# HKPolyU-UAV/bluerov2

Hardware: AMD Instinct MI355X
Metric: NMPC RTI solves/s (N=20, 12 states / 4 inputs), batch 4096 per GPU (higher is better)
Workload: dtype f64; 1 GPU; BASELINE.json configs[1]: batch=4096 independent BlueROV2 NMPC instances per GPU, N=20, Ts=0.05 s, circle reference window advancing one row per step, per-instance x0 noise (seed 1), nominal parameters, default options (qp_early_exit=1: exact equality-constrained shortcut when no bound is active); batch_per_gpu=4096, N=20, parallelism=single GPU

## Files before the change

bluerov2_amd/csrc/lin_device.hpp:

```cpp
#pragma once
#include "bluerov2_model.hpp"
#include "nmpc_device.hpp"

namespace brov {

__device__ __forceinline__ void kkt_upd(double& kkt, double v) {
    const double a = fabs(v);
    kkt = (a != a) ? a : ((kkt != kkt) ? kkt : fmax(kkt, a));
}

struct KktAcc {
    double mx = 0.0;
    bool nan = false;
    __device__ __forceinline__ void upd(double v) { mx = fmax(mx, fabs(v)); nan = nan || (v != v); }
};

__device__ __forceinline__ void rk4_state(const double* __restrict__ xi, const Wrench& w, const ModelPar& m, double h,
                                          StagePoint (&sp)[4], double (&xn)[NX]) {
    double x[NX], k[NX], xs[NX];
#pragma unroll
    for (int j = 0; j < NX; j++) x[j] = xi[j];
    model_f(x, w, m, k, sp[0]);
#pragma unroll
    for (int j = 0; j < NX; j++) { xn[j] = x[j] + (h / 6.0) * k[j]; xs[j] = x[j] + 0.5 * h * k[j]; }
// ... 107 lines not shown
    jvp_rec2(R, m.imx, m.imy, m.imz, m.imn, s0, s1, k0, k1);
#pragma unroll
    for (int st = 1; st < 4; st++) {
        R = load_stage_rec(rec + st * kRecStage);
        __builtin_amdgcn_sched_barrier(0);
        const double wprev = (st == 1) ? h / 6.0 : h / 3.0, cs = (st == 3) ? h : 0.5 * h;
#pragma unroll
        for (int j = 0; j < NX; j++) {
            const double e0 = (j == c0) ? 1.0 : 0.0, e1 = (j == c1) ? 1.0 : 0.0;
            acc0[j] = (st == 1 ? e0 : acc0[j]) + wprev * k0[j]; s0[j] = e0 + cs * k0[j];
            acc1[j] = (st == 1 ? e1 : acc1[j]) + wprev * k1[j]; s1[j] = e1 + cs * k1[j];
        }
        __builtin_amdgcn_sched_barrier(0);
        jvp_rec2(R, m.imx, m.imy, m.imz, m.imn, s0, s1, k0, k1);
    }
#pragma unroll
    for (int j = 0; j < NX; j++) { acc0[j] += (h / 6.0) * k0[j]; acc1[j] += (h / 6.0) * k1[j]; }
}

struct KktOperands { double pm1c, ll, lu, ucur, lbu, ubu, grad, qn; };
struct KktGlobal { double pm1c, ll, lu, ucur; };
__device__ __forceinline__ KktGlobal load_kkt_global(const DevParams& P, int b, int ig, int c, const double* __restrict__ ui) {
    const int N = P.N;
    const int jc = c - NX, ju = jc & 3, cx = c < NX ? c : NX - 1;
    const double* __restrict__ pim1 = P.pi + ((size_t)b * N + (ig > 0 ? ig - 1 : 0)) * NX;
    const double* __restrict__ lam = P.lam + ((size_t)b * N + ig) * 8;
    KktGlobal G;
    G.pm1c = pim1[cx];
    G.ll = lam[ju];
    G.lu = lam[4 + ju];
    G.ucur = ui[ju];
    return G;
}
__device__ __forceinline__ KktOperands finish_kkt_operands(const KktGlobal& G, const double* __restrict__ cst, int il, int nl, int c,
                                                           const lds_f64* q_s, const lds_f64* r_s) {
    const int jc = c - NX, ju = jc & 3, cx = c < NX ? c : NX - 1;
    KktOperands K;
    K.pm1c = G.pm1c; K.ll = G.ll; K.lu = G.lu; K.ucur = G.ucur;
    K.lbu = cst[32 + ju];
    K.ubu = cst[36 + ju];
    const lds_f64* gp = jc < 0 ? q_s + il * NX + c : r_s + il * NU + jc;
    K.grad = *gp;
    K.qn = q_s[nl * NX + cx];
    return K;
}
__device__ __forceinline__ KktOperands load_kkt_operands(const DevParams& P, const double* __restrict__ cst, int b, int ig, int il,
                                                         int nl, int c, const double* __restrict__ ui, const lds_f64* q_s,
                                                         const lds_f64* r_s) {
    return finish_kkt_operands(load_kkt_global(P, b, ig, c, ui), cst, il, nl, c, q_s, r_s);
}

__device__ __forceinline__ void sens_column_rec(const lds_f64* rec, const ModelPar& m, double h, int c, double (&acc)[NX]) {
    double ks[NX], ss[NX], kb[4];
    const int jc = c - NX;
    constexpr double ir = 1.0 / kRotor;
    kb[0] = jc == 0 ? (-4.0 * 0.707) * ir * m.imx : 0.0;
    kb[1] = jc == 1 ? (4.0 * 0.707) * ir * m.imy : 0.0;
    kb[2] = jc == 2 ? -2.0 * ir * m.imz : 0.0;
    kb[3] = jc == 1 ? (0.167 + 0.167 - 0.175 - 0.175) * ir * m.imn : (jc == 3 ? (0.167 + 0.167 + 0.175 + 0.175) * ir * m.imn : 0.0);
    StageRec R = load_stage_rec(rec);
    __builtin_amdgcn_sched_barrier(0);
#pragma unroll
    for (int j = 0; j < NX; j++) ss[j] = (j == c) ? 1.0 : 0.0;
    jvp_rec(R, m.imx, m.imy, m.imz, m.imn, kb, ss, ks);
    R = load_stage_rec(rec + kRecStage);
    __builtin_amdgcn_sched_barrier(0);
#pragma unroll
    for (int j = 0; j < NX; j++) { acc[j] = ((j == c) ? 1.0 : 0.0) + (h / 6.0) * ks[j]; ss[j] = ((j == c) ? 1.0 : 0.0) + 0.5 * h * ks[j]; }
    __builtin_amdgcn_sched_barrier(0);
    jvp_rec(R, m.imx, m.imy, m.imz, m.imn, kb, ss, ks);
    R = load_stage_rec(rec + 2 * kRecStage);
    __builtin_amdgcn_sched_barrier(0);
#pragma unroll
    for (int j = 0; j < NX; j++) { acc[j] += (h / 3.0) * ks[j]; ss[j] = ((j == c) ? 1.0 : 0.0) + 0.5 * h * ks[j]; }
    __builtin_amdgcn_sched_barrier(0);
    jvp_rec(R, m.imx, m.imy, m.imz, m.imn, kb, ss, ks);
    R = load_stage_rec(rec + 3 * kRecStage);
    __builtin_amdgcn_sched_barrier(0);
#pragma unroll
    for (int j = 0; j < NX; j++) { acc[j] += (h / 3.0) * ks[j]; ss[j] = ((j == c) ? 1.0 : 0.0) + h * ks[j]; }
    __builtin_amdgcn_sched_barrier(0);
    jvp_rec(R, m.imx, m.imy, m.imz, m.imn, kb, ss, ks);
// ... 116 lines not shown
```

bluerov2_amd/csrc/qp/fused.hpp:

```cpp
#pragma once

namespace brov {

constexpr int kFusedMaxN = 23;
template <int W, bool GRID, bool DF>
__device__ __forceinline__ bool rti_fused_step(const DevParams& P, int b, int lane, bool listed, size_t yoff) {
    extern __shared__ __attribute__((aligned(16))) double smem[];
    const int N = P.N;
    double* ba_s = smem;
    double* bv_s = ba_s + (size_t)N * kBaStage;
    double* kt_s = bv_s + (size_t)N * NX;
    double* kff_s = kt_s + (size_t)N * kKtStage;
    double* vh_s = kff_s + (size_t)N * 4;
    double* dx_s = vh_s + (size_t)N * 4;
    double* q_s = dx_s + (size_t)(N + 1) * NX;
    double* r_s = q_s + (size_t)(N + 1) * NX;
    double* const_s = r_s + (size_t)N * 4;
    if (lane == 0) { const_s[0] = 0.0; const_s[1] = 1.0; }
    LaneCst lc;
    if constexpr (W == 1) lc = load_lane_cst(P.cst, lane);
    double part = 0.0;
    bool nanp = false;
    lin_phase<W == 1, GRID>(P, b, 0, N, lane, ba_s, bv_s, kt_s, q_s, r_s, part, nanp, true, yoff);
    __syncthreads();
    if (P.dump_lin) copy_out_linearisation(P, b, 0, N, lane, ba_s, bv_s);
    std::conditional_t<GRID, InstGrid, Inst> I;
    setup_inst(P, I, b, lane, W == 1 ? &lc : nullptr, yoff);
    const bool listed_u = __builtin_amdgcn_readfirstlane((int)listed) != 0;
    I.ckpt = (N >= 8 && P.partial_refactor && listed_u) ? (N + 3) >> 2 : 0;
    I.lds_ba = (const lds_f64*)ba_s;
    I.lds_bv = (const lds_f64*)bv_s;
    I.lds_kt = (lds_f64*)kt_s;
    I.lds_q = (const lds_f64*)q_s;
    I.lds_r = (const lds_f64*)r_s;
    I.kff = kff_s;
    I.vhat = vh_s;
    I.dxb = dx_s;
    I.lds_kff = (lds_f64*)kff_s;
    I.lds_vhat = (lds_f64*)vh_s;
    I.lds_dxb = (lds_f64*)dx_s;
    I.lds_zero = (lds_f64*)const_s;
    I.lds_tr = (lds_f64*)const_s + 2;
    {
        const int rg = I.rg, cl = I.cl;
        const int zero = (int)(const_s - ba_s), one = zero + 1, kt0 = (int)(kt_s - ba_s);
        for (int r = 0; r < 3; r++) I.ba_off[r] = cl >= 3 ? (rg + 4 * r) * kBaStride + cl - 3 : ((r == 0 && rg == cl) ? one : zero);
        I.ba_str = cl >= 3 ? kBaStage : 0;
        for (int r = 0; r < 4; r++) {
            const int c = rg + 4 * r;
            I.bat_off[r] = cl >= NX ? zero : (c >= 3 ? cl * kBaStride + c - 3 : (c == cl ? one : zero));
        }
        I.bat_str = cl >= NX ? 0 : kBaStage;
        I.bat_str0 = (cl < NX && rg == 3) ? kBaStage : 0;
        for (int r = 0; r < 3; r++) I.kt_off[r] = cl < 4 ? kt0 + (rg + 4 * r) * 4 + cl : zero;
        I.kt_str = cl < 4 ? kKtStage : 0;
    }
    qp_body<W, std::conditional_t<GRID, InstGrid, Inst>, DF>(P, I, b, part, nanp);
    return I.ran_loop;
}
__device__ __forceinline__ void plant_step_wave(const DevParams& P, int b, int lane, int tk) {
    double x[NX], u[NU], k[NX], xs[NX], acc[NX];
    double* x0 = P.x0_rw + (size_t)b * NX;
#pragma unroll
    for (int j = 0; j < NX; j++) x[j] = x0[j];
#pragma unroll
    for (int j = 0; j < NU; j++) u[j] = P.res[b].u0[j];
    const ModelPar m = make_par(P.plant_pp + (size_t)b * NP);
    Wrench w = make_wrench(u);
    if (P.plant_rp) { w.k3 = P.plant_rp[(size_t)b * P.plant_rp_stride]; w.k4 = P.plant_rp[(size_t)b * P.plant_rp_stride + 1]; }
    const double h = P.plant_dt / P.plant_substeps;
    StagePoint sp;
    for (int s = 0; s < P.plant_substeps; s++) {
        model_f(x, w, m, k, sp);
#pragma unroll
        for (int j = 0; j < NX; j++) { acc[j] = x[j] + (h / 6.0) * k[j]; xs[j] = x[j] + 0.5 * h * k[j]; }
        model_f(xs, w, m, k, sp);
#pragma unroll
        for (int j = 0; j < NX; j++) { acc[j] += (h / 3.0) * k[j]; xs[j] = x[j] + 0.5 * h * k[j]; }
        model_f(xs, w, m, k, sp);
#pragma unroll
        for (int j = 0; j < NX; j++) { acc[j] += (h / 3.0) * k[j]; xs[j] = x[j] + h * k[j]; }
        model_f(xs, w, m, k, sp);
#pragma unroll
        for (int j = 0; j < NX; j++) x[j] = acc[j] + (h / 6.0) * k[j];
    }
    if (lane == 0) {
#pragma unroll
        for (int j = 0; j < NX; j++) x0[j] = x[j];
        if (P.plant_xlog) {
#pragma unroll
            for (int j = 0; j < NX; j++) P.plant_xlog[((size_t)tk * P.B + b) * NX + j] = x[j];
        }
        if (P.plant_ulog) {
#pragma unroll
            for (int j = 0; j < NU; j++) P.plant_ulog[((size_t)tk * P.B + b) * NU + j] = u[j];
        }
    }
}

template <int W, bool GRID = false, bool DF = false, bool MULTI = false>
__device__ __forceinline__ void rti_fused_body(const DevParams& P) {
    const int b = __builtin_amdgcn_readfirstlane(sched_map(P, blockIdx.x));
    const int lane = threadIdx.x;
    bool listed = sched_listed(P, b);
    if (blockIdx.x == 0) sched_zero_next(P, lane);
    DBG_STAMP(0);
    if constexpr (!MULTI) {
        (void)rti_fused_step<W, GRID, DF>(P, b, lane, listed, 0);
    } else {
#pragma clang loop unroll(disable)
        for (int tk = 0; tk < P.ticks; tk++) {
            int bq = b, lq = lane;
            asm volatile("s_mov_b32 %0, %0" : "+s"(bq));
            asm volatile("v_mov_b32 %0, %0" : "+v"(lq));
            listed = rti_fused_step<W, GRID, DF>(P, bq, lq, listed, (size_t)tk * (size_t)P.tick_yref);
            if (P.tick_status && lq == 0) P.tick_status[(size_t)tk * P.B + bq] = P.res[bq].status;
            __syncthreads();
            wave_fence();
            if (P.plant_pp) {
                plant_step_wave(P, bq, lq, tk);
                __syncthreads();
                wave_fence();
            }
        }
    }
}

}
```

bluerov2_amd/csrc/qp/lin_phase.hpp:

```cpp
#pragma once

namespace brov {

template <int MAXC>
__device__ __forceinline__ void stage_issue(const double* __restrict__ g, int nd, int lane, dbl2 (&v)[MAXC]) {
#pragma unroll
    for (int k = 0; k < MAXC; k++) {
        const int o = (lane + 64 * k) * 2;
        v[k] = *(const dbl2*)(g + (o < nd ? o : 0));
    }
}
template <int MAXC>
__device__ __forceinline__ void stage_store(double* l, int nd, int lane, const dbl2 (&v)[MAXC]) {
#pragma unroll
    for (int k = 0; k < MAXC; k++) {
        const int o = (lane + 64 * k) * 2;
        if (o < nd) *(lds_d2*)(l + o) = v[k];
    }
}

template <bool TWO = true, bool GRID = false>
__device__ __forceinline__ void lin_phase(const DevParams& P, int b, int i0, int n, int lane, double* ba_s, double* bv_s,
                                          double* rec_s, double* q_s, double* r_s, double& part, bool& nanp, bool stamp, size_t yoff = 0) {
#ifdef BROV_DBG_LIN
    unsigned long long lin_t[8] = {0, 0, 0, 0, 0, 0, 0, 0};
#endif
    const int N = P.N;
    const double* __restrict__ cst = P.cst;
    const int L = n <= 4 ? 16 : 64 / n;
    const int g = lane / L, j0 = lane - g * L;
    const bool active = g < n;
    const int i = active ? g : n - 1;
    const int ig = i0 + i;
    const double* __restrict__ ui = P.u + ((size_t)b * N + ig) * NU;
    const double hstep = GRID ? P.tsv[ig] : P.Ts;
    double rp0 = 0.0, rp1 = 0.0;
    if constexpr (TWO) {
        if (P.par_rp) { const double* rp = P.par_rp + ((size_t)b * (N + 1) + ig) * 2; rp0 = rp[0]; rp1 = rp[1]; }
    }
    const int po = i0 > 0 ? 1 : 0;
    double* sx = ba_s;
    double* spar = sx + (size_t)(n + 1) * NX;
    double* syr = spar + (size_t)n * NP;
    double* spi = syr + (size_t)(n + 1) * NY;
    double* su = spi + (size_t)(n + 1) * NX;
    {
        dbl2 vx[3], vp[3], vy[3], vpi[3], vu[1];
        stage_issue(P.x + ((size_t)b * (N + 1) + i0) * NX, (n + 1) * NX, lane, vx);
        stage_issue(P.par + ((size_t)b * (N + 1) + i0) * NP, n * NP, lane, vp);
        stage_issue(P.yref + yoff + (size_t)b * P.yref_stride + (size_t)i0 * NY, (n + 1) * NY, lane, vy);
        stage_issue(P.pi + ((size_t)b * N + i0 - po) * NX, (n + po) * NX, lane, vpi);
        stage_issue(P.u + ((size_t)b * N + i0) * NU, n * NU, lane, vu);
        stage_store(sx, (n + 1) * NX, lane, vx);
        stage_store(spar, n * NP, lane, vp);
        stage_store(syr, (n + 1) * NY, lane, vy);
        stage_store(spi, (n + po) * NX, lane, vpi);
        stage_store(su, n * NU, lane, vu);
    }
    const double* xi = sx + i * NX;
    const double* pp = spar + i * NP;
    const double* yr = syr + i * NY;
    const double* pil = spi + (i + po) * NX;
    const double* pim1 = spi + (ig > 0 ? i + po - 1 : 0) * NX;
    double uu[NU], x0r[NX], yrr[NY], pir[NX], pm1[3];
#pragma unroll
    for (int j = 0; j < NU; j++) uu[j] = su[i * NU + j];
#pragma unroll
    for (int j = 0; j < NX; j++) { x0r[j] = xi[j]; pir[j] = pil[j]; }
#pragma unroll
    for (int j = 0; j < NY; j++) yrr[j] = yr[j];
#pragma unroll
    for (int j = 0; j < 3; j++) pm1[j] = pim1[j];
    const unsigned long long tA = (stamp && P.dbg) ? __builtin_readcyclecounter() : 0;
    LIN_T(0);
    const bool last = ig == N - 1;
    double yrn[NX];
#pragma unroll
    for (int j = 0; j < NX; j++) yrn[j] = yr[NY + j];
    const ModelPar m = make_par(pp);
    Wrench w = make_wrench(uu);
    if constexpr (!TWO) {
        if (P.par_rp) { const double* rp = P.par_rp + ((size_t)b * (N + 1) + ig) * 2; rp0 = rp[0]; rp1 = rp[1]; }
    }
    w.k3 = rp0; w.k4 = rp1;
    KktAcc ka;
#pragma unroll
    for (int k = 0; k < NX; k++) {
        const double qk = (GRID ? P.wst[(size_t)ig * 16 + k] : P.Ts * cst[k]) * (x0r[k] - yrr[k]);
        q_s[i * NX + k] = qk;
        if (k < 3) ka.upd(ig >= 1 ? qk + pir[k] - pm1[k] : 0.0);
    }
#pragma unroll
    for (int k = 0; k < NU; k++) r_s[i * NU + k] = (GRID ? P.wst[(size_t)ig * 16 + NX + k] : P.Ts * cst[NX + k]) * (uu[k] - yrr[NX + k]);
    if (last) {
#pragma unroll
        for (int k = 0; k < NX; k++) {
            const double qn = cst[16 + k] * (xi[NX + k] - yrn[k]);
            q_s[n * NX + k] = qn;
            if (k < 3) ka.upd(qn - pir[k]);
        }
    }
    const unsigned long long tB = (stamp && P.dbg) ? __builtin_readcyclecounter() : 0;
    LIN_T(1);
    StagePoint sp[4];
    double xn[NX];
    rk4_state(x0r, w, m, hstep, sp, xn);
    const unsigned long long tC = (stamp && P.dbg) ? __builtin_readcyclecounter() : 0;
    LIN_T(2);
    double* tb = ba_s + i * kBaStage;
    lds_f64* rec = (lds_f64*)rec_s + i * kRecInterval;
#pragma unroll
    for (int st = 0; st < 4; st++) store_stage_rec(rec + st * kRecStage, sp[st], m);
#pragma unroll
    for (int k = 0; k < NX; k++) {
        const double bk = xn[k] - xi[NX + k];
        bv_s[i * NX + k] = bk;
        ka.upd(bk);
    }
    if (stamp && P.dbg && lane == 0)
        P.dbg[(size_t)b * 8 + 7] = ((tB - tA) & 0xFFFFF) | (((tC - tB) & 0xFFFFF) << 20) | (((__builtin_readcyclecounter() - tC) & 0xFFFFF) << 40);
    LIN_T(3);
    auto finish = [&](int c, const KktOperands& ko, const double (&acc)[NX]) __attribute__((always_inline)) {
        lin_kkt_col(ka, ko, N, ig, c, pir, acc);
#pragma unroll
        for (int k = 0; k < NX; k++) tb[k * kBaStride + (c - 3)] = acc[k];
    };
    if constexpr (TWO) {
#pragma unroll 1
        for (int q0 = j0; q0 - j0 < 6; q0 += 2 * L) {
            const int qa = q0 < 6 ? q0 : 5, qb = q0 + L < 6 ? q0 + L : 5;
            const int ca = qa < 3 ? 3 + qa : 6 + qa, cb = qb < 3 ? 3 + qb : 6 + qb;
            double acc0[NX], acc1[NX];
            const KktOperands koa = load_kkt_operands(P, cst, b, ig, i, n, ca, ui, (const lds_f64*)q_s, (const lds_f64*)r_s);
            const KktOperands kob = load_kkt_operands(P, cst, b, ig, i, n, cb, ui, (const lds_f64*)q_s, (const lds_f64*)r_s);
            sens_column_rec2(rec, m, hstep, ca, cb, acc0, acc1);
            finish(ca, koa, acc0);
            finish(cb, kob, acc1);
        }
    } else {
#pragma unroll 1
        for (int q0 = j0; q0 - j0 < 6; q0 += L) {
            const int qa = q0 < 6 ? q0 : 5;
            const int ca = qa < 3 ? 3 + qa : 6 + qa;
            double acc0[NX];
            const KktOperands koa = load_kkt_operands(P, cst, b, ig, i, n, ca, ui, (const lds_f64*)q_s, (const lds_f64*)r_s);
            sens_column_rec(rec, m, hstep, ca, acc0);
            finish(ca, koa, acc0);
        }
    }
    LIN_T(4);
    constexpr int kCheapTrips = 3;
    const int nC = (5 + L - 1) / L;
    KktGlobal kg[kCheapTrips];
    int cq[kCheapTrips];
#pragma unroll
    for (int t = 0; t < kCheapTrips; t++) {
        int q = j0 + t * L;
        q = q < 5 ? q : 4;
        cq[t] = q;
        const bool input = q >= 3;
        const int j = input ? (q == 3 ? 0 : 2) : q;
        kg[t] = load_kkt_global(P, b, ig, input ? NX + j : 6 + j, ui);
    }
#pragma unroll 1
    for (int q0 = j0; q0 - j0 < 2; q0 += L) {
        const int q = q0 < 2 ? q0 : 1;
        const int jc = 1 + 2 * q, c = NX + jc;
        double acc[NX];
        const KktOperands ko = load_kkt_operands(P, cst, b, ig, i, n, c, ui, (const lds_f64*)q_s, (const lds_f64*)r_s);
        sens_column_rec_u(rec, m, hstep, jc, acc);
        finish(c, ko, acc);
    }
    LIN_T(5);
    double cv[kCheapTrips][4];
#pragma unroll
    for (int t = 0; t < kCheapTrips; t++) {
        if (t < nC) {
            const int q = cq[t];
            const bool input = q >= 3;
            const int j = input ? (q == 3 ? 0 : 2) : q;
            constexpr double ir = 1.0 / kRotor;
            const double kbv = !input ? 0.0 : (j == 0 ? (-4.0 * 0.707) * ir * m.imx : -2.0 * ir * m.imz);
            sens_column_cheap(rec, hstep, j, input, kbv, cv[t]);
        }
    }
    LIN_T(6);
#pragma unroll
    for (int t = 0; t < kCheapTrips; t++) {
        if (t < nC) {
            const int q = cq[t];
            const bool input = q >= 3;
            const int j = input ? (q == 3 ? 0 : 2) : q;
            const int c = input ? NX + j : 6 + j;
            double acc[NX];
            expand_cheap(cv[t], j, acc);
            const double pr = (j == 0) ? pir[6] : ((j == 1) ? pir[7] : pir[8]);
            const double dotpi = cv[t][0] * pir[0] + cv[t][1] * pir[1] + cv[t][2] * pir[2] + cv[t][3] * pr;
            lin_kkt_rows(ka, finish_kkt_operands(kg[t], cst, i, n, c, (const lds_f64*)q_s, (const lds_f64*)r_s), N, ig, c, dotpi,
                         input ? 0.0 : pr);
#pragma unroll
            for (int k = 0; k < NX; k++) tb[k * kBaStride + (c - 3)] = acc[k];
        }
    }
    LIN_T(7);
#ifdef BROV_DBG_LIN
    if (stamp && P.dbg && lane == 0)
        for (int k = 0; k < 7; k++) P.dbg[(size_t)P.B * 8 + (size_t)b * 8 + (k == 6 ? 7 : k)] = lin_t[k + 1] - lin_t[k];
#endif
    if (active) {
        if (ka.nan) nanp = true;
        part = fmax(part, ka.mx);
    }
}

__device__ __forceinline__ void copy_out_linearisation(const DevParams& P, int b, int i0, int n, int lane, const double* ba_s,
                                                       const double* bv_s) {
    const int rg = lane >> 4, cl = lane & 15;
    const size_t g0 = (size_t)b * P.N + i0;
    for (int il = 0; il < n; il++) {
        const double* t = ba_s + il * kBaStage;
        double* BA = P.BA + (g0 + il) * 192;
#pragma unroll
        for (int r = 0; r < 3; r++) {
            const int row = rg + 4 * r;
            const double v = t[row * kBaStride + (cl >= 3 ? cl - 3 : 0)];
            const double m = cl >= 3 ? 1.0 : 0.0, c0 = (cl < 3 && row == cl) ? 1.0 : 0.0;
            BA[r * 64 + lane] = fma(m, v, c0);
        }
    }
    for (int j = lane; j < n * NX; j += 64) P.bvec[g0 * NX + j] = bv_s[j];
}
// ... 41 lines not shown
```

bluerov2_amd/csrc/qp/qp_body.hpp:

```cpp
#pragma once

namespace brov {

#define DBG_STAMP(slot) do { if (P.dbg && lane == 0) {                                                                          \
        P.dbg[(size_t)b * 8 + (slot)] = __builtin_readcyclecounter();                                                           \
        if ((slot) == 0) P.dbg[(size_t)P.B * 8 + (size_t)b * 8 + 7] = __builtin_amdgcn_s_memrealtime();                        \
        if ((slot) == 0) P.dbg[(size_t)P.B * 8 + (size_t)b * 8 + 5] = ((unsigned long long)__builtin_amdgcn_s_getreg(63508) << 32) | __builtin_amdgcn_s_getreg(63492); \
        if ((slot) == 6) P.dbg[(size_t)P.B * 8 + (size_t)b * 8 + 6] = __builtin_amdgcn_s_memrealtime(); } } while (0)
#ifdef BROV_DBG_IPM
#define IPM_T(k) do { const unsigned long long t_ = __builtin_readcyclecounter(); ipm_t[k] += t_ - ipm_last; ipm_last = t_; } while (0)
#else
#define IPM_T(k) do { } while (0)
#endif

#ifdef BROV_DBG_LIN
#define LIN_T(k) do { __builtin_amdgcn_sched_barrier(0); lin_t[k] = __builtin_readcyclecounter(); __builtin_amdgcn_sched_barrier(0); } while (0)
#else
#define LIN_T(k) do { } while (0)
#endif

template <int LDS, class IT = Inst, bool DF = false, bool LONGV = false>
__device__ __forceinline__ void qp_body(const DevParams& P, IT& I, int b, double lin_part, bool lin_nan, Win* W = nullptr,
                                        bool pre_ok = true, bool pre_illc = false) {
    constexpr bool EL = (LDS == 1 || LDS == 2);
    const double* __restrict__ cst = P.cst;
    const int lane = I.lane, N = I.NT, nv = I.nv;
    DBG_STAMP(1);
    const int rg = I.rg;

    double* x_it = P.x + (size_t)b * (N + 1) * 12;
    double* u_it = P.u + (size_t)b * N * 4;
    double* pi_it = P.pi + (size_t)b * N * 12;
    double* lam_it = P.lam + (size_t)b * N * 8;
    double* V = I.ipm + (size_t)IPM_V * nv;
    double* TL = I.ipm + (size_t)IPM_TL * nv;
    double* TU = I.ipm + (size_t)IPM_TU * nv;
    double* LL = I.ipm + (size_t)IPM_LL * nv;
    double* LU = I.ipm + (size_t)IPM_LU * nv;
    double* GAM = I.ipm + (size_t)IPM_GAM * nv;
    double* RT = I.ipm + (size_t)IPM_RT * nv;
    double* DVA = I.ipm + (size_t)IPM_DVA * nv;
    double* ACT = I.ipm + (size_t)IPM_ACT * nv;
    const double* GRAD = EL ? (const double*)I.kff : (const double*)DVA;
    auto rd_vhat = [&](int j) -> double { if constexpr (EL) return I.lds_vhat[j]; else return I.vhat[j]; };
    auto wr_vhat = [&](int j, double v) { if constexpr (EL) I.lds_vhat[j] = v; else I.vhat[j] = v; };
    auto rd_dxb = [&](int j) -> double { if constexpr (EL) return I.lds_dxb[j]; else return I.dxb[j]; };
    auto rd_grad = [&](int j) -> double { if constexpr (EL) return I.lds_kff[j]; else return GRAD[j]; };

    double x0v[3], xiv[3];
    {
        const double* x0 = P.x0 + (size_t)b * 12;
#pragma unroll
        for (int r = 0; r < 3; r++) { x0v[r] = x0[rg + 4 * r]; xiv[r] = I.x[rg + 4 * r]; }
    }
// ... 414 lines not shown
                if (unres <= P.tol_mu && rho <= P.tol_stat) converged = true;
                if (converged || (mu <= POL_MU_GATE * mu_gate && alpha >= POL_ALPHA_GATE)) { round_k = 0; round_cap = POL_LOOP; nchg_prev = nv + 1; }
            }
            if (converged && status == BROV_STATUS_MAXITER) status = BROV_STATUS_SUCCESS;
#ifdef BROV_DBG_IPM
            if (P.dbg && lane == 0) {
                ipm_t[6] = iters;
                for (int k = 0; k < 7; k++) P.dbg[(size_t)P.B * 8 + (size_t)b * 8 + k] = ipm_t[k];
            }
#endif
            use_vhat = polished || !ipm_on;
            if (!polished) {
                if (ipm_on) {
                    if constexpr (EL) { IPM_FOR(t, j) wr_vhat(j, vV.get(t, j)); }
                } else if (status == BROV_STATUS_MAXITER) {
                    GROUP_LANE;
                    IPM_PRE(up, I.u[j]);
                    IPM_PRE(vh, I.vhat[j]);
                    IPM_FOR(t, j) {
                        const double uj = EL ? ureg[t & 1] : (CACHE ? up[CACHE ? t : 0] : I.u[j]);
                        double vj = CACHE ? vh[CACHE ? t : 0] : rd_vhat(j);
                        vj = fmin(fmax(vj, lbI - uj), ubI - uj);
                        if constexpr (EL) wr_vhat(j, vj); else I.vhat[j] = vj;
                    }
                }
            }
#undef IPM_FOR
#undef IPM_PRE
#undef GROUP_LANE
        }
    }

    bool emitted = false;
    auto emit_record = [&](double cost_lane, double u0_lane, bool have_u0) __attribute__((always_inline)) {
        const double cs = wave_sum(cost_lane);
        if (lane == 0) {
            brov_result* r = P.res + b;
            r->cost = cs;
            r->kkt = kkt;
            r->status = status;
            r->qp_iter = early ? 0 : iters;
        }
        double u0r = u0_lane;
        if (!have_u0 && lane < 4) {
            u0r = P.res[b].u0[lane];
            u0r = (u0r == u0r) ? u0r : 0.0;
            u0r = fmin(fmax(u0r, cst[32 + lane]), cst[36 + lane]);
            P.res[b].u0[lane] = u0r;
        }
        const double a0 = readlane_f64(u0r, 0), a1 = readlane_f64(u0r, 1), a2 = readlane_f64(u0r, 2), a3 = readlane_f64(u0r, 3);
        const double s0 = (lane == 0 || lane == 1) ? -a0 : a0;
        const double s1 = (lane == 0 || lane == 2) ? a1 : -a1;
        const double s3 = (lane == 0 || lane == 3) ? a3 : -a3;
        const double th = ((lane < 4) ? (s0 + s1) + s3 : -a2) / kRotor;
        if (lane < 6) P.res[b].thrust[lane] = th;
        if (P.mail) {
            brov_result* m = P.mail + b;
            if (lane < 4) m->u0[lane] = u0r;
            if (lane < 6) m->thrust[lane] = th;
            if (lane == 0) { m->cost = cs; m->kkt = kkt; m->status = status; m->qp_iter = early ? 0 : iters; }
            if (P.mail_flag) {
                __threadfence_system();
                if (lane == 0) __hip_atomic_store(P.mail_flag + b, P.mail_seq, __ATOMIC_RELEASE, __HIP_MEMORY_SCOPE_SYSTEM);
            }
        }
        emitted = true;
    };

    constexpr int UX = EL ? 5 : 4, UU = EL ? 2 : 4;
    const double* vfin = (early || EL || use_vhat) ? I.vhat : V;
    const int nxe = (N + 1) * 12;
    double cost = 0.0;
    bool wrote_u0 = false;
    double u0v = 0.0;
    if (status == BROV_STATUS_SUCCESS || status == BROV_STATUS_MAXITER) {
        if (!early && !polished) {
            sw_rollout<LDS>(I, W, d0, vfin);
        }
        DBG_STAMP(4);
        if constexpr (LDS >= 3) {
            if (W->nan) {
                status = BROV_STATUS_NAN;
            } else {
                win_adjoint_commit<LDS == 4>(P, I, *W, b, vfin, early, cost, u0v, P.mail != nullptr && P.mail_early != 0,
                                             [&](double cost_lane, double u0_lane) __attribute__((always_inline)) { emit_record(cost_lane, u0_lane, true); });
                wrote_u0 = true;
            }
            DBG_STAMP(5);
        } else {
        double xpre[UX], ypre[UX], urpre[UU];
        double wxpre[LDS == 1 ? UX : 1], wupre[LDS == 1 ? UU : 1];
        if constexpr (EL) {
#pragma unroll
            for (int t = 0; t < UX; t++) {
                const int j = lane + 64 * t;
                const int jj = j < nxe ? j : 0;
                const int i = div12(jj), c = jj - i * 12;
                xpre[t] = x_it[jj];
                ypre[t] = I.yref[(size_t)i * 16 + c];
                if constexpr (LDS == 1) wxpre[t] = cst[(i == N) ? 16 + c : c];
            }
#pragma unroll
            for (int t = 0; t < UU; t++) {
                const int j = lane + 64 * t;
                const int jj = j < nv ? j : 0;
                urpre[t] = I.yref[(size_t)(jj >> 2) * 16 + 12 + (jj & 3)];
                if constexpr (LDS == 1) wupre[t] = cst[12 + (jj & 3)];
            }
        }
        auto copy_pi = [&]() __attribute__((always_inline)) {
            double pv5[5];
#pragma unroll
            for (int t = 0; t < 5; t++) pv5[t] = I.lds_kt[lane + 64 * t < N * 12 ? lane + 64 * t : 0];
#pragma unroll
            for (int t = 0; t < 5; t++) asm volatile("" : "+v"(pv5[t]));
#pragma unroll
            for (int t = 0; t < 5; t++)
                if (lane + 64 * t < N * 12) pi_it[lane + 64 * t] = pv5[t];
        };
        const bool late = DF && EL && early && P.mail != nullptr;
        if (!(EL && polished) && !late) sw_adjoint<true, LDS>(I, W, vfin, DVA, pi_it);
        DBG_STAMP(5);
        bool nanv = false;
        double vvp[EL ? UU : 1], djp[EL ? UX : 1];
        if constexpr (EL) {
#pragma unroll
            for (int t = 0; t < UU; t++) vvp[t] = rd_vhat(lane + 64 * t < nv ? lane + 64 * t : 0);
#pragma unroll
            for (int t = 0; t < UX; t++) djp[t] = rd_dxb(lane + 64 * t < nxe ? lane + 64 * t : 0);
#pragma unroll
            for (int t = 0; t < UU; t++) nanv = nanv || !(vvp[t] == vvp[t]);
#pragma unroll
            for (int t = 0; t < UX; t++) nanv = nanv || !(djp[t] == djp[t]);
        } else {
            for (int j = lane; j < nv; j += 64) {
                const double vj = vfin[j];
                if (!(vj == vj)) nanv = true;
            }
            for (int j = lane; j < nxe; j += 64) {
                const double dj = rd_dxb(j);
                if (!(dj == dj)) nanv = true;
            }
        }
        if (__ballot(nanv) != 0ull) {
            status = BROV_STATUS_NAN;
        } else {
            for (int j0 = lane; j0 < nv; j0 += 64 * UU) {
                double uo[UU], vv[UU], gg[UU], ur[UU];
#pragma unroll
                for (int t = 0; t < UU; t++) {
                    const int j = j0 + 64 * t;
                    const bool in = j < nv;
                    const int jj = in ? j : 0;
                    uo[t] = (EL && j0 == lane && t < 2) ? ureg[t] : u_it[jj];
                    vv[t] = EL ? ((j0 == lane) ? vvp[EL ? t : 0] : rd_vhat(jj)) : vfin[jj];
                    gg[t] = early ? 0.0 : rd_grad(jj);
                    ur[t] = (EL && j0 == lane) ? urpre[t] : I.yref[(size_t)(jj >> 2) * 16 + 12 + (jj & 3)];
                }
#pragma unroll
                for (int t = 0; t < UU; t++) {
                    const int j = j0 + 64 * t;
                    if (j < nv) {
                        const int i = j >> 2, m = j & 3;
                        lam_it[i * 8 + m] = gg[t] > 0 ? gg[t] : 0.0;
                        lam_it[i * 8 + 4 + m] = gg[t] < 0 ? -gg[t] : 0.0;
                        const double un = uo[t] + vv[t];
                        u_it[j] = un;
                        if (j < 4) { P.res[b].u0[j] = un; u0v = un; }
                        const double e = un - ur[t];
                        const double wgt = (LDS == 1 && j0 == lane) ? wupre[LDS == 1 ? t : 0] : cst[12 + m];
                        const double sw = (IT::kGrid || (LDS == 0 && I.wst)) ? I.wst[(size_t)i * 16 + 12 + m] : P.Ts * wgt;
                        cost += 0.5 * sw * e * e;
                    }
                }
            }
            wrote_u0 = true;
            if constexpr (EL) {
                if (!late) copy_pi();
            }
            for (int j0 = lane; j0 < nxe; j0 += 64 * UX) {
                double xo[UX], dj[UX], yr[UX];
#pragma unroll
                for (int t = 0; t < UX; t++) {
                    const int j = j0 + 64 * t;
                    const int jj = j < nxe ? j : 0;
                    const int i = div12(jj), c = jj - i * 12;
                    xo[t] = (EL && j0 == lane) ? xpre[t] : x_it[jj];
                    dj[t] = (EL && j0 == lane) ? djp[EL ? t : 0] : rd_dxb(jj);
                    yr[t] = (EL && j0 == lane) ? ypre[t] : I.yref[(size_t)i * 16 + c];
                }
#pragma unroll
                for (int t = 0; t < UX; t++) {
                    const int j = j0 + 64 * t;
                    if (j < nxe) {
                        const int i = div12(j), c = j - i * 12;
                        const double xn = xo[t] + dj[t];
                        x_it[j] = xn;
                        const double e = xn - yr[t];
                        const double wgt = (LDS == 1 && j0 == lane) ? wxpre[LDS == 1 ? t : 0] : cst[(i == N) ? 16 + c : c];
                        const double sw = (IT::kGrid || (LDS == 0 && I.wst)) ? I.wst[(size_t)i * 16 + c] : ((i == N) ? wgt : P.Ts * wgt);
                        cost += 0.5 * sw * e * e;
                    }
                }
            }
        }
        if constexpr (DF && EL) {
            if (late && status == BROV_STATUS_SUCCESS) {
                emit_record(cost, u0v, wrote_u0);
                sw_adjoint<true, LDS>(I, W, vfin, DVA, pi_it);
                copy_pi();
            } else if (late) {
            }
        }
        }
    }
    if (status != BROV_STATUS_SUCCESS && status != BROV_STATUS_MAXITER) {
        const double* x0 = P.x0 + (size_t)b * 12;
        const double xl = x0[lane < 12 ? lane : 0];
        const bool restart = P.on_failure == BROV_ON_FAILURE_RESTART && __ballot(!(fabs(xl) < 1e300)) == 0ull;
        for (int j = lane; j < nv; j += 64) {
            const int i = j >> 2, m = j & 3;
            const double e = u_it[j] - I.yref[(size_t)i * 16 + 12 + m];
            cost += 0.5 * ((IT::kGrid || (LDS == 0 && I.wst)) ? I.wst[(size_t)i * 16 + 12 + m] : P.Ts * cst[12 + m]) * e * e;
            if (restart) { u_it[j] = 0.0; lam_it[i * 8 + m] = 0.0; lam_it[i * 8 + 4 + m] = 0.0; }
        }
        for (int j = lane; j < nxe; j += 64) {
            const int i = j / 12, c = j - i * 12;
            const double e = x_it[j] - I.yref[(size_t)i * 16 + c];
            cost += 0.5 * ((IT::kGrid || (LDS == 0 && I.wst)) ? I.wst[(size_t)i * 16 + c] : ((i == N) ? cst[16 + c] : P.Ts * cst[c])) * e * e;
            if (restart) { x_it[j] = x0[c]; if (i < N) pi_it[j] = 0.0; }
        }
    }
    if (!emitted) emit_record(cost, u0v, wrote_u0);
#ifdef BROV_SCHED_TICKET_LATE
    if (sched_p == -2) sched_p = sched_ticket(P, b);
#endif
    sched_note(P, b, sched_p);
    I.ran_loop = !early;
    DBG_STAMP(6);
}


struct LaneCst { double Wr[4], Wer[3], lbm, ubm, Wq, Weq, Wuq; };
__device__ __forceinline__ LaneCst load_lane_cst(const double* __restrict__ cst, int lane) {
    const int rg = lane >> 4;
    LaneCst c;
#pragma unroll
    for (int r = 0; r < 4; r++) c.Wr[r] = cst[rg + 4 * r];
#pragma unroll
    for (int r = 0; r < 3; r++) c.Wer[r] = cst[16 + rg + 4 * r];
    c.lbm = cst[32 + rg];
    c.ubm = cst[36 + rg];
    const int cq = (lane >> 2) < NX ? (lane >> 2) : NX - 1;
    c.Wq = cst[cq];
    c.Weq = cst[16 + cq];
    c.Wuq = cst[12 + ((lane >> 2) & 3)];
    return c;
}
__device__ __forceinline__ void setup_inst(const DevParams& P, Inst& I, int b, int lane, const LaneCst* pre = nullptr, size_t yoff = 0) {
    const int N = P.N, nv = 4 * N;
    const double* __restrict__ cst = P.cst;
    I.lane = lane; I.rg = lane >> 4; I.cl = lane & 15; I.N = N; I.nv = nv;
    I.i0 = 0; I.NT = N; I.ckpt = 0;
    I.x = P.x + (size_t)b * (N + 1) * 12;
    I.u = P.u + (size_t)b * N * 4;
    I.yref = P.yref + yoff + (size_t)b * P.yref_stride;
    I.BA = P.BA + (size_t)b * N * 192;
    I.bvec = P.bvec + (size_t)b * N * 12;
    I.Ks = P.Ks + (size_t)b * N * 64;
    I.Kt = P.Kt + (size_t)b * N * 192;
// ... 30 lines not shown
```

bluerov2_amd/csrc/qp/sched.hpp:

```cpp
#pragma once

namespace brov {

template <int MODE, int T>
struct IpmVec {
    double r[T];
    double* g;
    __device__ __forceinline__ double get(int t, int j) const { return MODE ? r[t % T] : g[j]; }
    __device__ __forceinline__ void set(int t, int j, double v) { if (MODE) r[t % T] = v; else g[j] = v; }
    __device__ __forceinline__ void fetch(int lane, int nv) {
        if constexpr (MODE == 2) {
#pragma unroll
            for (int t = 0; t < T; t++) { const unsigned j = (unsigned)lane + 64u * t; r[t] = g[j < (unsigned)nv ? j : 0u]; }
        }
    }
    __device__ __forceinline__ void flush(int lane, int nv) const {
        if constexpr (MODE == 2) {
#pragma unroll
            for (int t = 0; t < T; t++) { const unsigned j = (unsigned)lane + 64u * t; if (j < (unsigned)nv) g[j] = r[t]; }
        }
    }
};

constexpr int kSchedClasses = 64, kSchedCntStride = 32;
// ... 24 lines not shown
}
__device__ __forceinline__ int wave_atomic_inc(int32_t* addr_uniform) {
    int ret = 0;
    const int zero = 0, one = 1;
    unsigned long long saved;
    asm volatile(
        "s_mov_b64 %[sv], exec\n\t"
        "s_mov_b64 exec, 1\n\t"
        "global_atomic_add %[r], %[off], %[one], %[base] sc0\n\t"
        "s_waitcnt vmcnt(0)\n\t"
        "s_mov_b64 exec, %[sv]"
        : [r] "+v"(ret), [sv] "=&s"(saved)
        : [off] "v"(zero), [one] "v"(one), [base] "s"(addr_uniform)
        : "memory");
    return __builtin_amdgcn_readfirstlane(ret);
}
__device__ __forceinline__ int sched_ticket(const DevParams& P, int b) {
    if (!P.sched) return -1;
    int32_t* Wr = (int32_t*)uniform_ptr(P.sched + (size_t)P.sched_w * P.sched_stride);
    return wave_atomic_inc(Wr + (b & (kSchedClasses - 1)) * kSchedCntStride);
}
__device__ __forceinline__ void sched_note(const DevParams& P, int b, int p) {
    if (!P.sched) return;
    int32_t* Wr = (int32_t*)uniform_ptr(P.sched + (size_t)P.sched_w * P.sched_stride);
    const int Bc = sched_class_len(P.B), k = b & (kSchedClasses - 1);
    if (p >= 0 && p < Bc) Wr[kSchedClasses * kSchedCntStride + k * Bc + p] = b;
    Wr[kSchedClasses * kSchedCntStride + kSchedClasses * Bc + b] = p;
}
__device__ __forceinline__ bool sched_listed(const DevParams& P, int b) {
    if (!P.sched) return true;
    const int32_t* Rd = uniform_ptr(P.sched + (size_t)P.sched_r * P.sched_stride);
    return Rd[kSchedClasses * kSchedCntStride + kSchedClasses * sched_class_len(P.B) + b] >= 0;
}
__device__ __forceinline__ void sched_zero_next(const DevParams& P, int lane) {
    if (P.sched && lane < kSchedClasses) P.sched[(size_t)P.sched_z * P.sched_stride + lane * kSchedCntStride] = 0;
}

}
```

Baseline: 5.754 million solves/s.

## Prefetch weights/bounds early and defer QP iterate stores to kernel tail

For the W==1 non-grid non-DF fused path, cost weights and input bounds are loaded into registers before the staging loads, and the listed flag is kept as a raw int so its load latency is not forced early. The QP result writeback (u, lambda, pi, x iterates) is held in registers and stored after the result record and scheduler bookkeeping, after a waitcnt, so global stores do not stall the critical path. This raises register pressure and relies on a single chunk per array, which is guarded by static_asserts on kFusedMaxN.

New measurement: 5.718 million solves/s. About the same (-0.6%).

```diff
diff --git a/bluerov2_amd/csrc/lin_device.hpp b/bluerov2_amd/csrc/lin_device.hpp
--- a/bluerov2_amd/csrc/lin_device.hpp
+++ b/bluerov2_amd/csrc/lin_device.hpp
@@ -163,13 +163,21 @@
     G.ucur = ui[ju];
     return G;
 }
-__device__ __forceinline__ KktOperands finish_kkt_operands(const KktGlobal& G, const double* __restrict__ cst, int il, int nl, int c,
+struct KktBounds { double lbu, ubu; };
+__device__ __forceinline__ KktBounds load_kkt_bounds(const double* __restrict__ cst, int c) {
+    const int ju = (c - NX) & 3;
+    KktBounds Bd;
+    Bd.lbu = cst[32 + ju];
+    Bd.ubu = cst[36 + ju];
+    return Bd;
+}
+__device__ __forceinline__ KktOperands finish_kkt_operands(const KktGlobal& G, const KktBounds& Bd, int il, int nl, int c,
                                                            const lds_f64* q_s, const lds_f64* r_s) {
-    const int jc = c - NX, ju = jc & 3, cx = c < NX ? c : NX - 1;
+    const int jc = c - NX, cx = c < NX ? c : NX - 1;
     KktOperands K;
     K.pm1c = G.pm1c; K.ll = G.ll; K.lu = G.lu; K.ucur = G.ucur;
-    K.lbu = cst[32 + ju];
-    K.ubu = cst[36 + ju];
+    K.lbu = Bd.lbu;
+    K.ubu = Bd.ubu;
     const lds_f64* gp = jc < 0 ? q_s + il * NX + c : r_s + il * NU + jc;
     K.grad = *gp;
     K.qn = q_s[nl * NX + cx];
@@ -178,7 +186,7 @@
 __device__ __forceinline__ KktOperands load_kkt_operands(const DevParams& P, const double* __restrict__ cst, int b, int ig, int il,
                                                          int nl, int c, const double* __restrict__ ui, const lds_f64* q_s,
                                                          const lds_f64* r_s) {
-    return finish_kkt_operands(load_kkt_global(P, b, ig, c, ui), cst, il, nl, c, q_s, r_s);
+    return finish_kkt_operands(load_kkt_global(P, b, ig, c, ui), load_kkt_bounds(cst, c), il, nl, c, q_s, r_s);
 }
 
 __device__ __forceinline__ void sens_column_rec(const lds_f64* rec, const ModelPar& m, double h, int c, double (&acc)[NX]) {
diff --git a/bluerov2_amd/csrc/qp/fused.hpp b/bluerov2_amd/csrc/qp/fused.hpp
--- a/bluerov2_amd/csrc/qp/fused.hpp
+++ b/bluerov2_amd/csrc/qp/fused.hpp
@@ -3,8 +3,10 @@
 namespace brov {
 
 constexpr int kFusedMaxN = 23;
-template <int W, bool GRID, bool DF>
-__device__ __forceinline__ bool rti_fused_step(const DevParams& P, int b, int lane, bool listed, size_t yoff) {
+static_assert(4 * kFusedMaxN <= 64 * 2 && 12 * kFusedMaxN <= 64 * 5 && 12 * (kFusedMaxN + 1) <= 64 * 5, "kFusedMaxN");
+template <int W, bool GRID, bool DF> constexpr bool kFusedLate = W == 1 && !GRID && !DF;
+template <int W, bool GRID, bool DF, class LT>
+__device__ __forceinline__ bool rti_fused_step(const DevParams& P, int b, int lane, LT listed, size_t yoff) {
     extern __shared__ __attribute__((aligned(16))) double smem[];
     const int N = P.N;
     double* ba_s = smem;
@@ -21,12 +23,18 @@
     if constexpr (W == 1) lc = load_lane_cst(P.cst, lane);
     double part = 0.0;
     bool nanp = false;
-    lin_phase<W == 1, GRID>(P, b, 0, N, lane, ba_s, bv_s, kt_s, q_s, r_s, part, nanp, true, yoff);
+    lin_phase<W == 1, GRID, kFusedLate<W, GRID, DF>>(P, b, 0, N, lane, ba_s, bv_s, kt_s, q_s, r_s, part, nanp, true, yoff);
     __syncthreads();
     if (P.dump_lin) copy_out_linearisation(P, b, 0, N, lane, ba_s, bv_s);
     std::conditional_t<GRID, InstGrid, Inst> I;
     setup_inst(P, I, b, lane, W == 1 ? &lc : nullptr, yoff);
-    const bool listed_u = __builtin_amdgcn_readfirstlane((int)listed) != 0;
+    bool listed_u;
+    if constexpr (std::is_same_v<LT, bool>) {
+        listed_u = __builtin_amdgcn_readfirstlane((int)listed) != 0;
+    } else {
+        asm volatile("" : "+v"(listed));
+        listed_u = __builtin_amdgcn_readfirstlane(listed) >= 0;
+    }
     I.ckpt = (N >= 8 && P.partial_refactor && listed_u) ? (N + 3) >> 2 : 0;
     I.lds_ba = (const lds_f64*)ba_s;
     I.lds_bv = (const lds_f64*)bv_s;
@@ -55,7 +63,7 @@
         for (int r = 0; r < 3; r++) I.kt_off[r] = cl < 4 ? kt0 + (rg + 4 * r) * 4 + cl : zero;
         I.kt_str = cl < 4 ? kKtStage : 0;
     }
-    qp_body<W, std::conditional_t<GRID, InstGrid, Inst>, DF>(P, I, b, part, nanp);
+    qp_body<W, std::conditional_t<GRID, InstGrid, Inst>, DF, false, kFusedLate<W, GRID, DF>>(P, I, b, part, nanp);
     return I.ran_loop;
 }
 __device__ __forceinline__ void plant_step_wave(const DevParams& P, int b, int lane, int tk) {
@@ -102,18 +110,21 @@
 __device__ __forceinline__ void rti_fused_body(const DevParams& P) {
     const int b = __builtin_amdgcn_readfirstlane(sched_map(P, blockIdx.x));
     const int lane = threadIdx.x;
-    bool listed = sched_listed(P, b);
+    constexpr bool LATE = kFusedLate<W, GRID, DF>;
+    std::conditional_t<LATE, int, bool> listed;
+    if constexpr (LATE) listed = sched_listed_word(P, b); else listed = sched_listed(P, b);
     if (blockIdx.x == 0) sched_zero_next(P, lane);
     DBG_STAMP(0);
     if constexpr (!MULTI) {
-        (void)rti_fused_step<W, GRID, DF>(P, b, lane, listed, 0);
+        (void)rti_fused_step<W, GRID, DF>(P, b, lane, listed, (size_t)0);
     } else {
 #pragma clang loop unroll(disable)
         for (int tk = 0; tk < P.ticks; tk++) {
             int bq = b, lq = lane;
             asm volatile("s_mov_b32 %0, %0" : "+s"(bq));
             asm volatile("v_mov_b32 %0, %0" : "+v"(lq));
-            listed = rti_fused_step<W, GRID, DF>(P, bq, lq, listed, (size_t)tk * (size_t)P.tick_yref);
+            const bool ran = rti_fused_step<W, GRID, DF>(P, bq, lq, listed, (size_t)tk * (size_t)P.tick_yref);
+            if constexpr (LATE) listed = ran ? 0 : -1; else listed = ran;
             if (P.tick_status && lq == 0) P.tick_status[(size_t)tk * P.B + bq] = P.res[bq].status;
             __syncthreads();
             wave_fence();
diff --git a/bluerov2_amd/csrc/qp/lin_phase.hpp b/bluerov2_amd/csrc/qp/lin_phase.hpp
--- a/bluerov2_amd/csrc/qp/lin_phase.hpp
+++ b/bluerov2_amd/csrc/qp/lin_phase.hpp
@@ -19,7 +19,7 @@
     }
 }
 
-template <bool TWO = true, bool GRID = false>
+template <bool TWO = true, bool GRID = false, bool PRE = false>
 __device__ __forceinline__ void lin_phase(const DevParams& P, int b, int i0, int n, int lane, double* ba_s, double* bv_s,
                                           double* rec_s, double* q_s, double* r_s, double& part, bool& nanp, bool stamp, size_t yoff = 0) {
 #ifdef BROV_DBG_LIN
@@ -44,6 +44,15 @@
     double* syr = spar + (size_t)n * NP;
     double* spi = syr + (size_t)(n + 1) * NY;
     double* su = spi + (size_t)(n + 1) * NX;
+    constexpr bool PREW = PRE && !GRID;
+    double cw[PREW ? 16 : 1], cwe[PREW ? NX : 1];
+    if constexpr (PREW) {
+#pragma unroll
+        for (int k = 0; k < 16; k++) cw[k] = cst[k];
+#pragma unroll
+        for (int k = 0; k < NX; k++) cwe[k] = cst[16 + k];
+        __builtin_amdgcn_sched_barrier(0);
+    }
     {
         dbl2 vx[3], vp[3], vy[3], vpi[3], vu[1];
         stage_issue(P.x + ((size_t)b * (N + 1) + i0) * NX, (n + 1) * NX, lane, vx);
@@ -57,6 +66,12 @@
         stage_store(spi, (n + po) * NX, lane, vpi);
         stage_store(su, n * NU, lane, vu);
     }
+    if constexpr (PREW) {
+#pragma unroll
+        for (int k = 0; k < 16; k++) asm volatile("" : "+v"(cw[k]));
+#pragma unroll
+        for (int k = 0; k < NX; k++) asm volatile("" : "+v"(cwe[k]));
+    }
     const double* xi = sx + i * NX;
     const double* pp = spar + i * NP;
     const double* yr = syr + i * NY;
@@ -86,16 +101,17 @@
     KktAcc ka;
 #pragma unroll
     for (int k = 0; k < NX; k++) {
-        const double qk = (GRID ? P.wst[(size_t)ig * 16 + k] : P.Ts * cst[k]) * (x0r[k] - yrr[k]);
+        const double qk = (GRID ? P.wst[(size_t)ig * 16 + k] : P.Ts * (PREW ? cw[PREW ? k : 0] : cst[k])) * (x0r[k] - yrr[k]);
         q_s[i * NX + k] = qk;
         if (k < 3) ka.upd(ig >= 1 ? qk + pir[k] - pm1[k] : 0.0);
     }
 #pragma unroll
-    for (int k = 0; k < NU; k++) r_s[i * NU + k] = (GRID ? P.wst[(size_t)ig * 16 + NX + k] : P.Ts * cst[NX + k]) * (uu[k] - yrr[NX + k]);
+    for (int k = 0; k < NU; k++)
+        r_s[i * NU + k] = (GRID ? P.wst[(size_t)ig * 16 + NX + k] : P.Ts * (PREW ? cw[PREW ? NX + k : 0] : cst[NX + k])) * (uu[k] - yrr[NX + k]);
     if (last) {
 #pragma unroll
         for (int k = 0; k < NX; k++) {
-            const double qn = cst[16 + k] * (xi[NX + k] - yrn[k]);
+            const double qn = (PREW ? cwe[PREW ? k : 0] : cst[16 + k]) * (xi[NX + k] - yrn[k]);
             q_s[n * NX + k] = qn;
             if (k < 3) ka.upd(qn - pir[k]);
         }
@@ -152,6 +168,7 @@
     constexpr int kCheapTrips = 3;
     const int nC = (5 + L - 1) / L;
     KktGlobal kg[kCheapTrips];
+    KktBounds kb[PRE ? kCheapTrips : 1];
     int cq[kCheapTrips];
 #pragma unroll
     for (int t = 0; t < kCheapTrips; t++) {
@@ -161,6 +178,7 @@
         const bool input = q >= 3;
         const int j = input ? (q == 3 ? 0 : 2) : q;
         kg[t] = load_kkt_global(P, b, ig, input ? NX + j : 6 + j, ui);
+        if constexpr (PRE) kb[t] = load_kkt_bounds(cst, input ? NX + j : 6 + j);
     }
 #pragma unroll 1
     for (int q0 = j0; q0 - j0 < 2; q0 += L) {
@@ -196,7 +214,8 @@
             expand_cheap(cv[t], j, acc);
             const double pr = (j == 0) ? pir[6] : ((j == 1) ? pir[7] : pir[8]);
             const double dotpi = cv[t][0] * pir[0] + cv[t][1] * pir[1] + cv[t][2] * pir[2] + cv[t][3] * pr;
-            lin_kkt_rows(ka, finish_kkt_operands(kg[t], cst, i, n, c, (const lds_f64*)q_s, (const lds_f64*)r_s), N, ig, c, dotpi,
+            const KktBounds kbt = PRE ? kb[PRE ? t : 0] : load_kkt_bounds(cst, c);
+            lin_kkt_rows(ka, finish_kkt_operands(kg[t], kbt, i, n, c, (const lds_f64*)q_s, (const lds_f64*)r_s), N, ig, c, dotpi,
                          input ? 0.0 : pr);
 #pragma unroll
             for (int k = 0; k < NX; k++) tb[k * kBaStride + (c - 3)] = acc[k];
diff --git a/bluerov2_amd/csrc/qp/qp_body.hpp b/bluerov2_amd/csrc/qp/qp_body.hpp
--- a/bluerov2_amd/csrc/qp/qp_body.hpp
+++ b/bluerov2_amd/csrc/qp/qp_body.hpp
@@ -19,7 +19,7 @@
 #define LIN_T(k) do { } while (0)
 #endif
 
-template <int LDS, class IT = Inst, bool DF = false, bool LONGV = false>
+template <int LDS, class IT = Inst, bool DF = false, bool LONGV = false, bool TAIL = false>
 __device__ __forceinline__ void qp_body(const DevParams& P, IT& I, int b, double lin_part, bool lin_nan, Win* W = nullptr,
                                         bool pre_ok = true, bool pre_illc = false) {
     constexpr bool EL = (LDS == 1 || LDS == 2);
@@ -500,27 +500,33 @@
     }
 
     bool emitted = false;
-    auto emit_record = [&](double cost_lane, double u0_lane, bool have_u0) __attribute__((always_inline)) {
-        const double cs = wave_sum(cost_lane);
-        if (lane == 0) {
+    double rec_cs = 0.0, rec_u0r = 0.0, rec_th = 0.0;
+    auto emit_record = [&](double cost_lane, double u0_lane, bool have_u0, int part = 0) __attribute__((always_inline)) {
+        if (part != 2) rec_cs = wave_sum(cost_lane);
+        if (part != 1 && lane == 0) {
             brov_result* r = P.res + b;
-            r->cost = cs;
+            r->cost = rec_cs;
             r->kkt = kkt;
             r->status = status;
             r->qp_iter = early ? 0 : iters;
         }
-        double u0r = u0_lane;
-        if (!have_u0 && lane < 4) {
-            u0r = P.res[b].u0[lane];
-            u0r = (u0r == u0r) ? u0r : 0.0;
-            u0r = fmin(fmax(u0r, cst[32 + lane]), cst[36 + lane]);
-            P.res[b].u0[lane] = u0r;
-        }
-        const double a0 = readlane_f64(u0r, 0), a1 = readlane_f64(u0r, 1), a2 = readlane_f64(u0r, 2), a3 = readlane_f64(u0r, 3);
-        const double s0 = (lane == 0 || lane == 1) ? -a0 : a0;
-        const double s1 = (lane == 0 || lane == 2) ? a1 : -a1;
-        const double s3 = (lane == 0 || lane == 3) ? a3 : -a3;
-        const double th = ((lane < 4) ? (s0 + s1) + s3 : -a2) / kRotor;
+        if (part != 2) {
+            double u0r = u0_lane;
+            if (!have_u0 && lane < 4) {
+                u0r = P.res[b].u0[lane];
+                u0r = (u0r == u0r) ? u0r : 0.0;
+                u0r = fmin(fmax(u0r, cst[32 + lane]), cst[36 + lane]);
+                P.res[b].u0[lane] = u0r;
+            }
+            const double a0 = readlane_f64(u0r, 0), a1 = readlane_f64(u0r, 1), a2 = readlane_f64(u0r, 2), a3 = readlane_f64(u0r, 3);
+            const double s0 = (lane == 0 || lane == 1) ? -a0 : a0;
+            const double s1 = (lane == 0 || lane == 2) ? a1 : -a1;
+            const double s3 = (lane == 0 || lane == 3) ? a3 : -a3;
+            rec_th = ((lane < 4) ? (s0 + s1) + s3 : -a2) / kRotor;
+            rec_u0r = u0r;
+        }
+        if (part == 1) return;
+        const double cs = rec_cs, u0r = rec_u0r, th = rec_th;
         if (lane < 6) P.res[b].thrust[lane] = th;
         if (P.mail) {
             brov_result* m = P.mail + b;
@@ -540,6 +546,8 @@
     const int nxe = (N + 1) * 12;
     double cost = 0.0;
     bool wrote_u0 = false;
+    bool tail_pending = false, tail_pi = false;
+    double tl_u[TAIL ? UU : 1], tl_ll[TAIL ? UU : 1], tl_lu[TAIL ? UU : 1], tl_pi[TAIL ? 5 : 1], tl_x[TAIL ? UX : 1];
     double u0v = 0.0;
     if (status == BROV_STATUS_SUCCESS || status == BROV_STATUS_MAXITER) {
         if (!early && !polished) {
@@ -576,12 +584,20 @@
                 if constexpr (LDS == 1) wupre[t] = cst[12 + (jj & 3)];
             }
         }
-        auto copy_pi = [&]() __attribute__((always_inline)) {
+        auto copy_pi = [&](bool park) __attribute__((always_inline)) {
             double pv5[5];
 #pragma unroll
             for (int t = 0; t < 5; t++) pv5[t] = I.lds_kt[lane + 64 * t < N * 12 ? lane + 64 * t : 0];
 #pragma unroll
             for (int t = 0; t < 5; t++) asm volatile("" : "+v"(pv5[t]));
+            if constexpr (TAIL) {
+                if (park) {
+#pragma unroll
+                    for (int t = 0; t < 5; t++) tl_pi[t] = pv5[t];
+                    tail_pi = true;
+                    return;
+                }
+            }
 #pragma unroll
             for (int t = 0; t < 5; t++)
                 if (lane + 64 * t < N * 12) pi_it[lane + 64 * t] = pv5[t];
@@ -630,21 +646,31 @@
                     const int j = j0 + 64 * t;
                     if (j < nv) {
                         const int i = j >> 2, m = j & 3;
-                        lam_it[i * 8 + m] = gg[t] > 0 ? gg[t] : 0.0;
-                        lam_it[i * 8 + 4 + m] = gg[t] < 0 ? -gg[t] : 0.0;
+                        if constexpr (TAIL) {
+                            tl_ll[t] = gg[t] > 0 ? gg[t] : 0.0;
+                            tl_lu[t] = gg[t] < 0 ? -gg[t] : 0.0;
+                        } else {
+                            lam_it[i * 8 + m] = gg[t] > 0 ? gg[t] : 0.0;
+                            lam_it[i * 8 + 4 + m] = gg[t] < 0 ? -gg[t] : 0.0;
+                        }
                         const double un = uo[t] + vv[t];
-                        u_it[j] = un;
-                        if (j < 4) { P.res[b].u0[j] = un; u0v = un; }
+                        if constexpr (TAIL) tl_u[t] = un; else u_it[j] = un;
+                        if (j < 4) {
+                            if constexpr (!TAIL) P.res[b].u0[j] = un;
+                            u0v = un;
+                        }
                         const double e = un - ur[t];
                         const double wgt = (LDS == 1 && j0 == lane) ? wupre[LDS == 1 ? t : 0] : cst[12 + m];
                         const double sw = (IT::kGrid || (LDS == 0 && I.wst)) ? I.wst[(size_t)i * 16 + 12 + m] : P.Ts * wgt;
                         cost += 0.5 * sw * e * e;
                     }
                 }
+                if constexpr (TAIL) break;
             }
             wrote_u0 = true;
+            if constexpr (TAIL) tail_pending = true;
             if constexpr (EL) {
-                if (!late) copy_pi();
+                if (!late) copy_pi(true);
             }
             for (int j0 = lane; j0 < nxe; j0 += 64 * UX) {
                 double xo[UX], dj[UX], yr[UX];
@@ -663,20 +689,21 @@
                     if (j < nxe) {
                         const int i = div12(j), c = j - i * 12;
                         const double xn = xo[t] + dj[t];
-                        x_it[j] = xn;
+                        if constexpr (TAIL) tl_x[t] = xn; else x_it[j] = xn;
                         const double e = xn - yr[t];
                         const double wgt = (LDS == 1 && j0 == lane) ? wxpre[LDS == 1 ? t : 0] : cst[(i == N) ? 16 + c : c];
                         const double sw = (IT::kGrid || (LDS == 0 && I.wst)) ? I.wst[(size_t)i * 16 + c] : ((i == N) ? wgt : P.Ts * wgt);
                         cost += 0.5 * sw * e * e;
                     }
                 }
+                if constexpr (TAIL) break;
             }
         }
         if constexpr (DF && EL) {
             if (late && status == BROV_STATUS_SUCCESS) {
                 emit_record(cost, u0v, wrote_u0);
                 sw_adjoint<true, LDS>(I, W, vfin, DVA, pi_it);
-                copy_pi();
+                copy_pi(false);
             } else if (late) {
             }
         }
@@ -699,11 +726,43 @@
             if (restart) { x_it[j] = x0[c]; if (i < N) pi_it[j] = 0.0; }
         }
     }
-    if (!emitted) emit_record(cost, u0v, wrote_u0);
+    if constexpr (!TAIL) {
+        if (!emitted) emit_record(cost, u0v, wrote_u0);
 #ifdef BROV_SCHED_TICKET_LATE
-    if (sched_p == -2) sched_p = sched_ticket(P, b);
+        if (sched_p == -2) sched_p = sched_ticket(P, b);
 #endif
-    sched_note(P, b, sched_p);
+        sched_note(P, b, sched_p);
+    } else {
+        static_assert(EL && UU == 2 && UX == 5, "one chunk per array (qp/fused.hpp checks kFusedMaxN against these)");
+        emit_record(cost, u0v, wrote_u0, 1);
+#ifdef BROV_SCHED_TICKET_LATE
+        if (sched_p == -2) sched_p = sched_ticket(P, b);
+#endif
+        __builtin_amdgcn_s_waitcnt(0x0F70);
+        emit_record(cost, u0v, wrote_u0, 2);
+        sched_note(P, b, sched_p);
+        if (tail_pending) {
+#pragma unroll
+            for (int t = 0; t < UU; t++) {
+                const int j = lane + 64 * t;
+                if (j < nv) {
+                    const int i = j >> 2, m = j & 3;
+                    lam_it[i * 8 + m] = tl_ll[t];
+                    lam_it[i * 8 + 4 + m] = tl_lu[t];
+                    u_it[j] = tl_u[t];
+                    if (j < 4) P.res[b].u0[j] = tl_u[t];
+                }
+            }
+            if (tail_pi) {
+#pragma unroll
+                for (int t = 0; t < 5; t++)
+                    if (lane + 64 * t < N * 12) pi_it[lane + 64 * t] = tl_pi[t];
+            }
+#pragma unroll
+            for (int t = 0; t < UX; t++)
+                if (lane + 64 * t < nxe) x_it[lane + 64 * t] = tl_x[t];
+        }
+    }
     I.ran_loop = !early;
     DBG_STAMP(6);
 }
diff --git a/bluerov2_amd/csrc/qp/sched.hpp b/bluerov2_amd/csrc/qp/sched.hpp
--- a/bluerov2_amd/csrc/qp/sched.hpp
+++ b/bluerov2_amd/csrc/qp/sched.hpp
@@ -80,6 +80,11 @@
     const int32_t* Rd = uniform_ptr(P.sched + (size_t)P.sched_r * P.sched_stride);
     return Rd[kSchedClasses * kSchedCntStride + kSchedClasses * sched_class_len(P.B) + b] >= 0;
 }
+__device__ __forceinline__ int sched_listed_word(const DevParams& P, int b) {
+    if (!P.sched) return 0;
+    const int32_t* Rd = uniform_ptr(P.sched + (size_t)P.sched_r * P.sched_stride);
+    return Rd[kSchedClasses * kSchedCntStride + kSchedClasses * sched_class_len(P.B) + b];
+}
 __device__ __forceinline__ void sched_zero_next(const DevParams& P, int lane) {
     if (P.sched && lane < kSchedClasses) P.sched[(size_t)P.sched_z * P.sched_stride + lane * kSchedCntStride] = 0;
 }
```
